# kellerberrin/KGL_Gene

Measured on AMD Instinct MI355X. Metric: variants·genomes/sec (allele-freq sweep), higher is better.
Workload: dtype u32

## Files before the change

### kgl_gene_amd/csrc/kgx_inbreed.hip

```cpp
#include <hip/hip_runtime.h>

#include <algorithm>
#include <cmath>
#include <cstdio>
#include <cstdlib>
#include <cstring>
#include <new>
#include <random>
#include <string>
#include <vector>

#include "kgx_kernels_inbreed.h"
#include "kgx_kernels_hall.h"
#include "kgx_kernels_loglik.h"
#include <hipcub/hipcub.hpp>
#include "kgx_internal.h"
#include "kgx_inbreed_plan.h"
#include "kgx_inbreed_buffers.h"

namespace kgx {
namespace {

int require_runtime(std::shared_ptr<Runtime>& rt) {
  rt = current_runtime();
  if (!rt) return fail(KGX_ENODEVICE, "kgx_init() has not succeeded: no gfx950 device bound (there is no CPU fallback)");
  return KGX_OK;
}

int sync_shards(const kgx_gt8* h) {
  for (const auto& sh : h->shards) {
    if (int rc = use_device(*sh.dev)) return rc;
    KGX_HIP(hipStreamSynchronize(sh.dev->stream));
  }
  return use_device(*h->shards[0].dev);
}

void destroy_shards(kgx_gt8* h) {
  for (auto& sh : h->shards)
    if ((sh.d_gt || sh.d_wide || sh.d_wide_of_row) && use_device(*sh.dev) == KGX_OK) {
      if (sh.d_gt) (void)hipFree(sh.d_gt);
      if (sh.d_wide) (void)hipFree(sh.d_wide);
      if (sh.d_wide_of_row) (void)hipFree(sh.d_wide_of_row);
      sh.d_gt = nullptr; sh.d_wide = nullptr; sh.d_wide_of_row = nullptr;
    }
  if (!h->shards.empty()) (void)use_device(*h->shards[0].dev);
}


static_assert(kAlgoSimple == KGX_ALGO_SIMPLE && kAlgoRitlandLocus == KGX_ALGO_RITLAND_LOCUS && kAlgoHallME == KGX_ALGO_HALL_ME &&
              kAlgoLoglikelihood == KGX_ALGO_LOGLIKELIHOOD, "the plan's algorithms are kgx.h's");

InbreedSwitches read_switches(int algorithm) {
  InbreedSwitches sw;
  sw.generic = env_int("KGX_K5_GENERIC", 0) != 0;
  sw.no_eval_lut = env_int("KGX_K5_NO_EVAL_LUT", 0) != 0;
  sw.no_table_sweep = env_int("KGX_K5_NO_TABLE_SWEEP", 0) != 0;
  sw.no_swar16 = env_int("KGX_K5_NO_SWAR16", 0) != 0;
  sw.eval_gpl = env_int("KGX_K5_EVAL_GPL", 8);
  if (sw.eval_gpl != 4 && sw.eval_gpl != 8) sw.eval_gpl = 8;
  sw.blocks_per_cu = env_int("KGX_K5_BLOCKS_PER_CU", 8);
  sw.eval_resident = env_int("KGX_K5_EVAL_RESIDENT", 2);
  sw.eval_rounds = env_int("KGX_K5_EVAL_ROUNDS", 8);
  sw.sequential_min = env_int("KGX_K5_SEQUENTIAL_MIN", 1 << 16);
  sw.always_guard = env_int("KGX_K5_ALWAYS_GUARD", 0) != 0;
  sw.xcds = static_cast<uint32_t>(std::max(1, env_int("KGX_K5_XCDS", 1)));
  sw.time_small_calls = env_int("KGX_TIME_SMALL_CALLS", 0) != 0;
  sw.keep_scratch_gb = env_int("KGX_KEEP_SCRATCH_GB", -1);
  sw.no_wave = env_int("KGX_K7_NO_WAVE", 0) != 0;
  sw.wave_loci = std::min(kGenomeWaveLoci, std::max(1, env_int("KGX_K7_WAVE_LOCI", 1024)));
  sw.wave_genomes = std::max(1, env_int("KGX_K7_WAVE_GENOMES", algorithm == KGX_ALGO_HALL_ME ? 1024 : 512));
  sw.search_brent = env_str("KGX_K7_SEARCH") == "brent";
  sw.hall_passes = env_int("KGX_K7_HALL_PASSES", 0) != 0;
  sw.golden = env_int("KGX_K7_GOLDEN", 0) != 0;
  sw.estimate_start = env_int("KGX_K7_ESTIMATE_START", 0);
  sw.ll_passes = env_int("KGX_K7_LL_PASSES", 0) != 0;
  sw.ll_het_terms = env_int("KGX_K7_LL_HET_TERMS", 0) != 0;
  sw.ll_dense_per_1024 = env_int("KGX_K7_LL_DENSE_PER_1024", 0);
  sw.class_sweeps = env_int("KGX_K7_CLASS_SWEEPS", 0) != 0;
  sw.class_bytes = env_int("KGX_K7_CLASS_BYTES", 0) != 0;
  sw.order_one_lane = env_int("KGX_K7_ORDER_ONE_LANE", 0) != 0;
  sw.no_pair = env_int("KGX_K7_NO_PAIR", 0) != 0;
  sw.no_compact = env_int("KGX_K7_NO_COMPACT", 0) != 0;
  sw.compact_min_genomes = env_int("KGX_K7_COMPACT_MIN_GENOMES", 2048);
  sw.compact_min_cells = env_int("KGX_K7_COMPACT_MIN_CELLS", 1 << 26);
  sw.trace = env_int("KGX_K7_TRACE", 0) != 0;
  return sw;
}

struct ClassHits {
  unsigned long long* words = nullptr;
  uint64_t word_blocks = 0;
  bool by_bits = false;
  HallClassRows class_rows{};
};

struct EvalTarget {
  const uint32_t* gt;
  uint64_t dwords_per_row, g0, n;
  const uint32_t* index;
  double* f;
};

struct InbreedCall;

struct ActiveSet {
  uint64_t n_act = 0, g0 = 0, dwords_per_row = 0;
  const uint32_t* gt = nullptr;
  const uint32_t* index = nullptr;
  BrentState* brent = nullptr;
  double* f = nullptr;
  uint32_t* d_global = nullptr;
  std::vector<uint32_t> global_of;
  std::vector<BrentState> host_states;
  bool may_compact_now = false;
  int compaction_level = 0;
  void compact(InbreedCall& c, unsigned int running, bool whatever_the_size);
};

struct InbreedCall {
  Device& dev;
  kgx_gt8_shard& sh;
  hipStream_t st;
  InbreedShape shape;
  InbreedSwitches sw;
  InbreedPlan plan;
  const uint32_t* locus_index;
  const double* minor_af;
  const double* start;
  kgx_locus_results* out;
  double* objective_out;
// ... 380 lines not shown
                             m.moments, block_bins, words_per_block, class_out, hits.word_blocks, static_cast<uint32_t>(block_base_of_class & 7u));
        });
      });
    } else {
      const dim3 sweep_grid(class_items[k] * hall_chunks);
      auto sweep = [&](auto gpl_c, auto emit_c) {
        hipLaunchKernelGGL((k_hall_sweep<decltype(gpl_c)::value, decltype(emit_c)::value>), sweep_grid, dim3(kBlock), 0, st, gt32, dwords_per_row, g0, n,
                           m.padded_of(k), m.items_of(k), h_counters + 4 * k, hall_chunks, code, m.moments, m.item_blocks_of(k), block_bins, words_per_block,
                           class_out);
      };
      if (plan.eval_gpl == 8) with_bool(emit, [&](auto emit_c) { sweep(std::integral_constant<int, 8>{}, emit_c); });
      else sweep(std::integral_constant<int, 4>{}, std::false_type{});
    }
    hipLaunchKernelGGL(k_hall_merge, dim3(hall_merge_blocks, 256), dim3(kBlock), 0, st, m.moments, item_base, n, m.bins, m.bin_used(), k + 1u);
    try_hip(hipGetLastError(), KGX_EHIP, "hall moments launch");
  }
  loglik_classes.n = emit ? hall_classes : 0u;
  loglik_classes.block_bins = block_bins;
  loglik_classes.plain_words = (by_bits && hall_mfma) ? 1u : 0u;
  loglik_classes.word_blocks = hits.word_blocks;
  loglik_classes.dense = sw.ll_dense_per_1024 > 0 ? sw.ll_dense_per_1024 / 1024.0 : kLoglikDense;
  try_hip(hipEventRecord(dev.moments_end, st), KGX_EHIP, "hipEventRecord");
  moments_timed = true;
  hipLaunchKernelGGL(k_hall_used_bins, dim3(1), dim3(kBlock), 0, st, m.bin_used(), m.used(), m.totals());
  try_hip(hipGetLastError(), KGX_EHIP, "hall bins launch");
  return rc == KGX_OK;
}

void InbreedCall::iterate_one_launch() {
  const uint64_t n = shape.n, n_sel = shape.n_sel;
  const bool hall = shape.algorithm == KGX_ALGO_HALL_ME;
  const bool per_wave = n_sel <= static_cast<uint64_t>(sw.wave_loci) && n >= static_cast<uint64_t>(sw.wave_genomes);
  const uint32_t wave_grid = static_cast<uint32_t>(per_wave ? (n + kBlock / kWave - 1) / (kBlock / kWave) : n);
  const double* estimate = hall ? b.d_sums : sw.estimate_start ? b.d_sums : nullptr;
  const int threads = per_wave ? kWave : kBlock;
  int cells = per_wave ? 8 : 2;
  while (cells < 32 && n_sel > static_cast<uint64_t>(threads) * cells) cells *= 2;
  with_int<1, 2>(hall ? 1 : 2, [&](auto mode_c) {
    auto launch = [&](auto cells_c, auto threads_c) {
      hipLaunchKernelGGL((k_inbreed_iterate_genome<decltype(mode_c)::value, decltype(cells_c)::value, decltype(threads_c)::value>), dim3(wave_grid), dim3(kBlock),
                         0, st, sh.d_gt, sh.pitch, shape.g0, n, d_index, n_sel, b.d_table, b.d_valid, shape.amax, shape.phased, b.d_counts, estimate, plan.search,
                         b.d_start, b.d_f, b.d_running);
    };
    if (per_wave) with_int<8, 16, 32>(cells, [&](auto cells_c) { launch(cells_c, std::integral_constant<int, kWave>{}); });
    else with_int<2, 4, 8, 16, 32>(cells, [&](auto cells_c) { launch(cells_c, std::integral_constant<int, kBlock>{}); });
  });
  wave_evaluations = !hall;
  dev.last_path = KGX_PATH_ONE_LAUNCH;
}

bool InbreedCall::hall_by_moments() {
  if (!(plan.hall_candidate && rc == KGX_OK && gather_moments(false))) return false;
  try_hip(hipEventRecord(dev.search_begin, st), KGX_EHIP, "hipEventRecord");
  hipLaunchKernelGGL(k_hall_iterate, dim3(static_cast<uint32_t>(shape.n)), dim3(kBlock), 0, st, m.bins, m.used(), m.totals(), b.d_counts, shape.n, b.d_start, b.d_f);
  try_hip(hipGetLastError(), KGX_EHIP, "hall iterate launch");
  try_hip(hipEventRecord(dev.search_end, st), KGX_EHIP, "hipEventRecord");
  search_timed = true;
  if (rc == KGX_OK) dev.last_path = KGX_PATH_HALL_MOMENTS;
  return rc == KGX_OK;
}

void InbreedCall::hall_by_passes() {
  const uint64_t n = shape.n, n_sel = shape.n_sel;
  if (rc == KGX_OK) dev.last_path = KGX_PATH_HALL_PASSES;
  const std::vector<double>& f0 = start_points;
  const unsigned long long walked =
      plan.eval_lut && n_sel ? (plan.eval_n_seg - 1) * plan.eval_per_seg + (n_sel - (plan.eval_n_seg - 1) * plan.eval_per_seg + 7) / 8 * 8 : 0ull;
  try_hip(hipMemcpyAsync(b.d_f, f0.data(), n * sizeof(double), hipMemcpyHostToDevice, st), KGX_EHIP, "H2D(f0)");
  try_hip(hipStreamSynchronize(st), KGX_EHIP, "sync");
  tabulate(1);
  std::vector<double> trace_prev, trace_prev2, trace_now;
  if (sw.trace) { trace_prev = f0; trace_prev2 = f0; trace_now.resize(n); }
  for (int it = 0; it < 50 && rc == KGX_OK; ++it) {
    estimator_pass(1, false);
    hipLaunchKernelGGL(k_reduce_parts, dim3(reduce_grid(n)), dim3(kBlock), 0, st, b.d_part, plan.pass_n_seg, n, nullptr, b.d_eval);
    hipLaunchKernelGGL(k_hall_update, dim3(lin_grid), dim3(kBlock), 0, st, b.d_eval, b.d_counts, n, walked, b.d_f);
    if (!sw.trace) continue;
    try_hip(hipMemcpyAsync(trace_now.data(), b.d_f, n * sizeof(double), hipMemcpyDeviceToHost, st), KGX_EHIP, "D2H(trace)");
    try_hip(hipStreamSynchronize(st), KGX_EHIP, "sync");
    uint64_t changed = 0, cycling = 0;
    double worst = 0.0;
    for (uint64_t g = 0; g < n; ++g) {
      if (trace_now[g] != trace_prev[g]) {
        ++changed;
        if (trace_now[g] == trace_prev2[g]) ++cycling;
        const double d = std::fabs(trace_now[g] - trace_prev[g]);
        worst = d > worst ? d : worst;
      }
    }
    std::fprintf(stderr, "[kgx] HallME step %d: %llu of %llu genomes moved (%llu back to the value before), largest move %.3e\n", it + 1,
                 (unsigned long long)changed, (unsigned long long)n, (unsigned long long)cycling, worst);
    trace_prev2 = trace_prev;
    trace_prev = trace_now;
  }
}

bool InbreedCall::loglik_by_moments(std::vector<uint32_t>& handed_over) {
  const uint64_t n = shape.n;
  const int objective_method = shape.objective_method;
  const bool loglik_moments = plan.loglik_candidate;
  if (objective_method == 1 && !loglik_moments)
    rc = fail(KGX_ESTATE, "kgx_inbreed_objective: this call would not run on the moments (selection size, amax, phase, memory or a switch)");
  if (!(loglik_moments && objective_method != 2 && rc == KGX_OK && gather_moments(true))) {
    if (objective_method == 1 && rc == KGX_OK)
      rc = fail(KGX_ESTATE, "kgx_inbreed_objective: a frequency without a bin, or no room for the hits' words: the passes would run");
    return false;
  }
  uint32_t* const h_totals = m.totals();
  uint32_t n_used = 0;
  try_hip(hipMemcpyAsync(&n_used, h_totals, sizeof(uint32_t), hipMemcpyDeviceToHost, st), KGX_EHIP, "D2H(used bins)");
  try_hip(hipStreamSynchronize(st), KGX_EHIP, "sync");
  unsigned long long* d_search_stats = sw.trace ? m.d_search_stats : nullptr;
  if (d_search_stats) try_hip(hipMemsetAsync(d_search_stats, 0, 8 * sizeof(unsigned long long), st), KGX_EHIP, "memset(search stats)");
  try_hip(hipEventRecord(dev.search_begin, st), KGX_EHIP, "hipEventRecord");
  hipLaunchKernelGGL(k_loglik_search, dim3(static_cast<uint32_t>(n)), dim3(kBlock), loglik_search_lds(n_used), st, m.bins, m.used(), h_totals, b.d_counts, b.d_sums,
                     m.d_smallest_het, n, plan.words_per_block, loglik_classes, b.d_start, objective_method == 1 ? 1 : 0, b.d_f, m.d_needs_passes, h_totals + 2,
                     b.d_running, d_search_stats);
  try_hip(hipGetLastError(), KGX_EHIP, "loglik search launch");
  try_hip(hipEventRecord(dev.search_end, st), KGX_EHIP, "hipEventRecord");
  search_timed = true;
  uint32_t handed = 0;
  unsigned int evaluations = 0;
  try_hip(hipMemcpyAsync(&handed, h_totals + 2, sizeof(uint32_t), hipMemcpyDeviceToHost, st), KGX_EHIP, "D2H(handed over)");
  try_hip(hipMemcpyAsync(&evaluations, b.d_running, sizeof(unsigned int), hipMemcpyDeviceToHost, st), KGX_EHIP, "D2H(evaluations)");
  try_hip(hipStreamSynchronize(st), KGX_EHIP, "sync");
  if (rc != KGX_OK) return false;
  if (d_search_stats) {
    unsigned long long stats[8] = {0};
    try_hip(hipMemcpy(stats, d_search_stats, sizeof(stats), hipMemcpyDeviceToHost), KGX_EHIP, "D2H(search stats)");
    std::fprintf(stderr, "kgx: Loglikelihood search over %llu genomes (%u bins used): %llu evaluations, %llu with cells in their band -- %llu served by kept cells, "
                         "%llu gathers kept, %llu gathers not kept, %llu dense walks; %llu cells listed, %llu blocks looked at\n",
                 (unsigned long long)n, n_used, stats[0], stats[1], stats[2], stats[3], stats[4], stats[5], stats[6], stats[7]);
  }
  dev.last_evaluations = static_cast<int>(evaluations);
  dev.last_path = KGX_PATH_LOGLIK_MOMENTS;
  if (handed) {
    std::vector<uint32_t> flags(n);
    try_hip(hipMemcpyAsync(flags.data(), m.d_needs_passes, n * sizeof(uint32_t), hipMemcpyDeviceToHost, st), KGX_EHIP, "D2H(needs passes)");
    try_hip(hipMemcpyAsync(b.d_keep, b.d_f, n * sizeof(double), hipMemcpyDeviceToDevice, st), KGX_EHIP, "copy(kept results)");
    try_hip(hipMemsetAsync(b.d_running, 0, sizeof(unsigned int), st), KGX_EHIP, "memset(running)");
    try_hip(hipStreamSynchronize(st), KGX_EHIP, "sync");
    for (uint64_t g = 0; g < n; ++g)
      if (flags[g]) {
        handed_over.push_back(static_cast<uint32_t>(g));
        if (sw.trace) std::fprintf(stderr, "kgx: Loglikelihood: genome %llu handed to the passes (reason %u)\n", (unsigned long long)(shape.g0 + g), flags[g]);
      }
    if (rc == KGX_OK) dev.last_path = KGX_PATH_LOGLIK_MOMENTS_AND_PASSES;
  }
  return true;
}

int InbreedCall::loglik_objective() {
  const uint64_t n = shape.n;
  if (shape.objective_method == 2 && rc == KGX_OK) {
    try_hip(hipMemcpyAsync(b.d_f, b.d_start, n * sizeof(double), hipMemcpyDeviceToDevice, st), KGX_EHIP, "copy(points)");
    tabulate(2);
    estimator_pass(2, false);
    hipLaunchKernelGGL(k_reduce_parts, dim3(reduce_grid(n)), dim3(kBlock), 0, st, b.d_part, plan.pass_n_seg, n, nullptr, b.d_eval);
    try_hip(hipGetLastError(), KGX_EHIP, "objective pass launch");
  }
  try_hip(hipMemcpyAsync(objective_out, shape.objective_method == 2 ? b.d_eval : b.d_f, n * sizeof(double), hipMemcpyDeviceToHost, st), KGX_EHIP, "D2H(objective)");
  try_hip(hipStreamSynchronize(st), KGX_EHIP, "sync");
  return rc;
}

void ActiveSet::compact(InbreedCall& c, unsigned int running, bool whatever_the_size) {
  Device& dev = c.dev;
  hipStream_t st = c.st;
  const uint64_t n_sel = c.shape.n_sel, planes = c.plan.planes;
  const uint64_t new_pitch = (static_cast<uint64_t>(running) + 127) / 128 * 128;
// ... 684 lines not shown
```

### kgl_gene_amd/csrc/kgx_inbreed_constants.h

```cpp
#ifndef KGX_INBREED_CONSTANTS_H
#define KGX_INBREED_CONSTANTS_H

#include <stdint.h>

#if defined(__HIPCC__)
#define KGX_HOST_DEVICE __host__ __device__
#else
#define KGX_HOST_DEVICE
#endif

namespace kgx {

constexpr int kWave = 64;
constexpr int kBlock = 256;

constexpr int kEvalBatch = 8;
constexpr uint64_t kRitlandSegment = 4088;

constexpr int kSearchBrent = 0, kSearchNelderMead = 1;
constexpr int kSearchNelderMeadPair = 2;

constexpr int kGenomeLoci = 8192;
constexpr int kGenomeWaveLoci = 2048;

constexpr int kHallMoments = 5;
constexpr int kHallKeyMantissa = 7;
constexpr int kHallMinExponent = -20;
constexpr uint32_t kHallBins = 1u + static_cast<uint32_t>(-kHallMinExponent) * (1u << kHallKeyMantissa) + 1u;
constexpr uint32_t kHallItemLoci = 2048;
struct HallRecord { uint32_t row; uint32_t bin; double delta; };
constexpr uint32_t kHallBlockLoci = 64;
constexpr uint64_t kBitsSpanGenomes = 2048;
constexpr uint64_t kBitsSpanBytes = kBitsSpanGenomes / 8;
KGX_HOST_DEVICE inline uint64_t hall_bit_row_bytes(uint64_t n_genomes) { return (n_genomes + kBitsSpanGenomes - 1) / kBitsSpanGenomes * kBitsSpanBytes; }

}

#endif
```

### kgl_gene_amd/csrc/kgx_inbreed_plan.h

```cpp
#ifndef KGX_INBREED_PLAN_H
#define KGX_INBREED_PLAN_H

#include <cassert>
#include <cstddef>
#include <stdint.h>

#include "kgx_inbreed_constants.h"

namespace kgx {

constexpr int kAlgoRitlandLocus = 0, kAlgoSimple = 1, kAlgoHallME = 2, kAlgoLoglikelihood = 3;

struct InbreedSwitches {
  bool generic = false;
  bool no_eval_lut = false;
  bool no_table_sweep = false;
  bool no_swar16 = false;
  int eval_gpl = 8;
  int blocks_per_cu = 8;
  int eval_resident = 2;
  int eval_rounds = 8;
  int sequential_min = 1 << 16;
  bool always_guard = false;
  uint32_t xcds = 1;
  bool time_small_calls = false;
  int keep_scratch_gb = -1;
  bool no_wave = false;
  int wave_loci = 1024;
  int wave_genomes = 1024;
  bool search_brent = false;
  bool hall_passes = false;
  bool golden = false;
  int estimate_start = 0;
  bool ll_passes = false;
  bool ll_het_terms = false;
  int ll_dense_per_1024 = 0;
  bool class_sweeps = false;
  bool class_bytes = false;
  bool order_one_lane = false;
  bool no_pair = false;
  bool no_compact = false;
  int compact_min_genomes = 2048;
  int compact_min_cells = 1 << 26;
  bool trace = false;
};

struct InbreedShape {
  uint64_t n = 0;
  uint64_t g0 = 0;
  uint64_t n_sel = 0;
  uint32_t amax = 1;
  int phased = 0;
  int algorithm = kAlgoSimple;
  int objective_method = 0;
  bool has_locus_index = false;
  int compute_units = 0;
};

struct InbreedPlan {
  bool ritland = false, table_sweep = false, swar16 = false, generic_sweep = false, eval_lut = false;
  int eval_gpl = 8;
  uint32_t gx = 0, gx16 = 0;
  uint64_t n_seg = 1, per_seg = 8, eval_n_seg = 1, eval_per_seg = 8, max_seg = 1, pass_n_seg = 1;
  bool sequential_defaults = false, wave_sized = false, table_passes = false;
  int search = kSearchNelderMead, pass_search = kSearchNelderMead;
  uint64_t planes = 1;
  bool hall_candidate = false, loglik_candidate = false;
  uint32_t hall_classes = 1;
  uint64_t hall_items = 0, hall_blocks = 0;
  uint64_t words_per_block = 0;
  bool hall_mfma = false, hall_bits_planned = false;
  bool hit_words_planned = false;
  uint64_t sel_pitch = 0, bit_row_bytes = 0;
  uint64_t moments_extra_bytes = 0;

  bool by_moments() const { return hall_candidate || loglik_candidate; }
  void take_the_passes() {
    hall_candidate = loglik_candidate = hall_mfma = hall_bits_planned = hit_words_planned = false;
    hall_items = hall_blocks = 0;
  }
};

inline InbreedPlan plan_inbreed(const InbreedShape& s, const InbreedSwitches& sw) {
  InbreedPlan p;
  const uint64_t n = s.n, g0 = s.g0, n_sel = s.n_sel;
  const uint32_t amax = s.amax;
  const uint64_t compute_units = static_cast<uint64_t>(s.compute_units);
  p.ritland = s.algorithm == kAlgoRitlandLocus;
  const bool no_tables = sw.generic || sw.no_eval_lut;
// ... 75 lines not shown
```

### kgl_gene_amd/csrc/kgx_kernels_hall.h

```cpp
#pragma once

#include <cstdint>

#include "kgx_kernels_inbreed.h"

namespace kgx {

constexpr uint32_t kHallNoKey = 0xFFFu;
constexpr int kHallBinsPerThread = (kHallBins + kBlock - 1) / kBlock;
static_assert(kHallBins < kHallNoKey, "12-bit sort keys");

struct HallItem { uint32_t begin, end, bin, pad; };
__host__ __device__ inline uint64_t hall_word_index(uint64_t block, uint64_t g, uint64_t lanes) {
  return ((block * 4 + ((g >> 1) & 3)) * lanes + (g >> 3)) * 2 + (g & 1);
}

__device__ __forceinline__ uint32_t hall_key(double y) {
  if (y == 0.0) return 0u;
  const uint64_t bits = static_cast<uint64_t>(__double_as_longlong(y));
  const int exponent = static_cast<int>((bits >> 52) & 0x7FFu) - 1023;
  if (!(y > 0.0) || exponent < kHallMinExponent || y > 1.0) return kHallNoKey;
  return 1u + static_cast<uint32_t>(exponent - kHallMinExponent) * (1u << kHallKeyMantissa) +
         static_cast<uint32_t>((bits >> (52 - kHallKeyMantissa)) & ((1u << kHallKeyMantissa) - 1u));
}
// ... 714 lines not shown
}

template <int BINS>
__device__ __forceinline__ double hall_iterate_genome(const double* __restrict__ bins, const uint32_t* __restrict__ used, uint32_t n_used,
                                                      uint64_t n_genomes, uint64_t g, double total, double F, double (&row_part)[2][16]) {
  double centre[BINS], m[BINS][kHallMoments];
#pragma unroll
  for (int i = 0; i < BINS; ++i) {
    const uint32_t at = threadIdx.x + static_cast<uint32_t>(i) * kBlock;
    centre[i] = 1.0;
#pragma unroll
    for (int j = 0; j < kHallMoments; ++j) m[i][j] = 0.0;
    if (at < n_used) {
      const uint32_t bin = used[at];
      centre[i] = hall_centre(bin);
#pragma unroll
      for (int j = 0; j < kHallMoments; ++j) m[i][j] = bins[(static_cast<uint64_t>(bin) * kHallMoments + j) * n_genomes + g];
    }
  }
  auto block_sum = [&](double v, int pass) {
    v = row_sum16(v);
    if ((threadIdx.x & 15) == 0) row_part[pass & 1][threadIdx.x >> 4] = v;
    __syncthreads();
    const double* p = row_part[pass & 1];
    double pair[8];
#pragma unroll
    for (int i = 0; i < 8; ++i) pair[i] = p[2 * i] + p[2 * i + 1];
    return ((pair[0] + pair[1]) + (pair[2] + pair[3])) + ((pair[4] + pair[5]) + (pair[6] + pair[7]));
  };
  for (int it = 0; it < 50; ++it) {
    const bool positive = F > 0.0;
    const double Fs = positive ? F : 1.0;
    const double u = 1.0 - Fs;
    double sum = 0.0;
#pragma unroll
    for (int i = 0; i < BINS; ++i) {
      const double q = 1.0 / __builtin_fma(u, centre[i], Fs);
      const double t = -u * q;
      double h = m[i][4];
      h = __builtin_fma(h, t, m[i][3]);
      h = __builtin_fma(h, t, m[i][2]);
      h = __builtin_fma(h, t, m[i][1]);
      h = __builtin_fma(h, t, m[i][0]);
      sum = __builtin_fma(q, h, sum);
    }
    const double S = block_sum(sum, it);
    F = positive ? (F * S) / total : 0.0 / total;
  }
  return F;
}

__global__ void __launch_bounds__(kBlock)
k_hall_iterate(const double* __restrict__ bins, const uint32_t* __restrict__ used, const uint32_t* __restrict__ n_used_ptr,
               const unsigned long long* __restrict__ counts, uint64_t n_genomes, const double* __restrict__ start, double* __restrict__ f_out) {
  __shared__ double row_part[2][16];
  const uint64_t g = blockIdx.x;
  if (g >= n_genomes) return;
  const uint32_t n_used = *n_used_ptr;
  const double total = static_cast<double>(counts[g * 6 + 4]);
  double F;
  if (n_used <= 4u * kBlock) F = hall_iterate_genome<4>(bins, used, n_used, n_genomes, g, total, start[g], row_part);
  else if (n_used <= 8u * kBlock) F = hall_iterate_genome<8>(bins, used, n_used, n_genomes, g, total, start[g], row_part);
  else F = hall_iterate_genome<kHallBinsPerThread>(bins, used, n_used, n_genomes, g, total, start[g], row_part);
  if (threadIdx.x == 0) f_out[g] = F;
}

}
```

### kgl_gene_amd/csrc/kgx_kernels_loglik.h

```cpp
#pragma once

#include <cstdint>

#include "kgx_kernels_hall.h"

namespace kgx {

constexpr int kLoglikTmaxLog2 = 4;
constexpr double kLoglikTmax = 1.0 / (1 << kLoglikTmaxLog2);
constexpr double kLoglikBand = 1.0 / (1.0 - (1.0 / 256.0) / kLoglikTmax);
constexpr double kLoglikReach = 0.5 * kLoglikBand * (1.0 + 1.0 / 64.0);
constexpr int kLoglikMaxClasses = 15;
constexpr uint32_t kLoglikListCells = 2560;
constexpr int kLoglikWordsPerThread = 4;
constexpr double kLoglikDense = 1.0 / 4.0;
constexpr double kLogSmallProb = -23.025850929940457;
constexpr int kLoglikBinValues = 6;

struct LoglikClass {
  const double* ys;
  const uint32_t* bin_block;
  const unsigned long long* words;
};
struct LoglikClasses { LoglikClass of[kLoglikMaxClasses]; uint32_t n; uint32_t block_bins; uint32_t plain_words; uint64_t word_blocks; double dense; };

inline size_t loglik_search_lds(uint32_t n_used) {
  return static_cast<size_t>(n_used) * (kLoglikBinValues * sizeof(double) + sizeof(uint32_t)) + 8;
}

__global__ void __launch_bounds__(kBlock)
k_loglik_search(const double* __restrict__ bins, const uint32_t* __restrict__ used, const uint32_t* __restrict__ n_used_ptr,
                const unsigned long long* __restrict__ counts, const double* __restrict__ sums,
                const unsigned long long* __restrict__ smallest_het, uint64_t n_genomes, uint64_t words_per_block, LoglikClasses classes,
                const double* __restrict__ start, int mode, double* __restrict__ f_out, uint32_t* __restrict__ needs_passes,
                uint32_t* __restrict__ handed_over, unsigned int* __restrict__ max_evaluations, unsigned long long* __restrict__ stats = nullptr) {
  extern __shared__ double bin_values[];
  __shared__ double row_part[2][3][16];
  __shared__ double cell_y[kLoglikListCells];
  __shared__ uint32_t wave_total[2][kBlock / kWave];
  const uint64_t g = blockIdx.x;
  if (g >= n_genomes) return;
  const uint32_t n_used = *n_used_ptr;
  uint32_t* const bin_keys = reinterpret_cast<uint32_t*>(bin_values + static_cast<size_t>(kLoglikBinValues) * n_used);
  for (uint32_t i = threadIdx.x; i < n_used; i += kBlock) {
    const uint32_t bin = used[i];
    const double* m = bins + static_cast<uint64_t>(bin) * kHallMoments * n_genomes + g;
    double v[kLoglikBinValues] = {m[0], 0.0, 0.0, 0.0, 0.0, 0.0};
    if (bin != 0u) {
      const double r = 1.0 / hall_centre(bin);
      v[1] = m[n_genomes]; v[2] = m[2 * n_genomes] * 0.5; v[3] = m[3 * n_genomes] * (1.0 / 3.0); v[4] = m[4 * n_genomes] * 0.25;
      v[5] = r * (v[1] - r * (v[2] - r * (v[3] - r * v[4])));
    }
#pragma unroll
    for (int j = 0; j < kLoglikBinValues; ++j) bin_values[static_cast<size_t>(j) * n_used + i] = v[j];
    bin_keys[i] = bin;
  }
  __syncthreads();
  const uint32_t wave = threadIdx.x / kWave, lane = threadIdx.x % kWave;
  const uint64_t lanes = words_per_block / 8;
  int pass = 0, scans = 0;
  auto block_sum3 = [&](double& a, double& b, double& c) {
    a = row_sum16(a);
    b = row_sum16(b);
    c = row_sum16(c);
    double (*slot)[16] = row_part[pass & 1];
    if ((threadIdx.x & 15) == 0) { slot[0][threadIdx.x >> 4] = a; slot[1][threadIdx.x >> 4] = b; slot[2][threadIdx.x >> 4] = c; }
    __syncthreads();
    double out[3];
#pragma unroll
    for (int which = 0; which < 3; ++which) {
      const double* p = slot[which];
      double pair[8];
#pragma unroll
      for (int i = 0; i < 8; ++i) pair[i] = p[2 * i] + p[2 * i + 1];
      out[which] = ((pair[0] + pair[1]) + (pair[2] + pair[3])) + ((pair[4] + pair[5]) + (pair[6] + pair[7]));
    }
    a = out[0]; b = out[1]; c = out[2];
    ++pass;
  };
  auto block_scan = [&](uint32_t mine, uint32_t& total) {
    uint32_t inclusive = mine;
#pragma unroll
    for (int off = 1; off < kWave; off <<= 1) {
      const uint32_t up = __shfl_up(inclusive, off);
      if (lane >= static_cast<uint32_t>(off)) inclusive += up;
    }
    uint32_t* totals = wave_total[scans & 1];
    if (lane == kWave - 1) totals[wave] = inclusive;
    __syncthreads();
    uint32_t before = 0;
    total = 0;
#pragma unroll
    for (uint32_t w = 0; w < kBlock / kWave; ++w) {
      if (w < wave) before += totals[w];
      total += totals[w];
    }
    ++scans;
    return before + inclusive - mine;
  };
  const unsigned long long sixth = counts[g * 6 + 5], total_cells = counts[g * 6 + 4];
  const double het_big = static_cast<double>(sixth >> 32);
  const double het_tiny = static_cast<double>(total_cells - (sixth & 0xFFFFFFFFull));
  const double het_cells = static_cast<double>(counts[g * 6 + 1] + counts[g * 6 + 3]) - het_tiny;
  const double het_term = sums[g * kParts0 + 4];
  const double w_smallest = __longlong_as_double(static_cast<long long>(*smallest_het));
  uint32_t hand_over = het_big != 0.0 ? 1u : 0u;

  auto band_of = [&](double F, uint32_t& key_lo, uint32_t& key_hi) {
    const double u = 1.0 - F;
    const double disc = sqrt(__builtin_fma(F, F, 4.0 * u * 1e-10));
    const double y_floor = u > 0.0 ? (F <= 0.0 ? (disc - F) / (2.0 * u) : 2e-10 / (F + disc)) : 1e-10;
    const double y_under = y_floor * (1.0 - 1e-9), y_over = y_floor * (1.0 + 1e-9);
    key_lo = y_under < 9.5367431640625e-07 ? 1u : hall_key(y_under);
    key_hi = y_over < 9.5367431640625e-07 ? 1u : hall_key(y_over) + 1u;
    const double edge = F < 0.0 ? -F / u * kLoglikBand : 0.0;
    if (edge >= 9.5367431640625e-07) {
      const uint32_t k_edge = hall_key(edge);
      const uint32_t from = hall_centre(k_edge) < edge ? k_edge + 1u : k_edge;
      key_hi = from > key_hi ? from : key_hi;
    }
  };
  uint32_t kept_lo = 0, kept_hi = 0, kept_n = 0;

  auto objective = [&](double F, double reach_lo, double reach_hi) -> double {
    const double u = 1.0 - F;
    uint32_t key_lo, key_hi, wide_lo, wide_hi, unused;
    band_of(F, key_lo, key_hi);
    band_of(reach_hi, wide_lo, unused);
    band_of(reach_lo, unused, wide_hi);
    wide_lo = wide_lo < key_lo ? wide_lo : key_lo;
    wide_hi = wide_hi > key_hi ? wide_hi : key_hi;
    double sum = 0.0, band_cells = 0.0, wide_cells = 0.0;
    for (uint32_t i = threadIdx.x; i < n_used; i += kBlock) {
      const uint32_t key = bin_keys[i];
      const double m0 = bin_values[i];
      if (key >= key_hi) {
        const double c = hall_centre(key);
        const double A = __builtin_fma(u, c, F), t = u / A;
        const double m1 = bin_values[n_used + i], m2 = bin_values[2 * n_used + i], m3 = bin_values[3 * n_used + i], m4 = bin_values[4 * n_used + i];
        sum += __builtin_fma(m0, log(c * A), bin_values[5 * n_used + i]) + t * (m1 - t * (m2 - t * (m3 - t * m4)));
      } else if (key < key_lo) {
        sum += m0 * kLogSmallProb;
      } else {
        band_cells += m0;
      }
      if (key >= wide_lo && key < wide_hi) wide_cells += m0;
    }
    block_sum3(sum, band_cells, wide_cells);
    double value = sum;
    if (stats && threadIdx.x == 0) { atomicAdd(stats + 0, 1ull); if (band_cells > 0.0) atomicAdd(stats + 1, 1ull); }
    if (band_cells > 0.0) {
      if (key_hi > classes.block_bins || wide_hi > classes.block_bins) hand_over = 2u;
      double prod = 1.0;
      int expo = 0;
      auto exact_cell = [&](double y) {
        const double yy = y * y, d = y - yy;
        const double p = __builtin_fmin(__builtin_fmax(__builtin_fma(F, d, yy), 0.0), 1.0);
        prod *= __builtin_fmax(p, 1e-10);
      };
      auto peel = [&]() {
        expo += __builtin_amdgcn_frexp_exp(prod);
        prod = __builtin_amdgcn_frexp_mant(prod);
      };
      const bool kept_covers = kept_hi != 0u && kept_lo <= key_lo && key_hi <= kept_hi;
      const bool keep = !kept_covers && wide_cells <= static_cast<double>(kLoglikListCells);
      const uint32_t from = keep ? wide_lo : key_lo, to = keep ? wide_hi : key_hi;
      uint32_t band_blocks = 0;
      if (!kept_covers)
        for (uint32_t k = 0; k < classes.n; ++k) band_blocks += classes.of[k].bin_block[to] - classes.of[k].bin_block[from];
      const bool dense = !kept_covers && !keep && band_cells >= classes.dense * static_cast<double>(band_blocks) * kHallBlockLoci;
      auto walk_listed = [&](uint32_t n_listed) {
        for (uint32_t i0 = 0; i0 < n_listed; i0 += 8 * kBlock) {
#pragma unroll
          for (int q = 0; q < 8; ++q) {
            const uint32_t i = i0 + static_cast<uint32_t>(q) * kBlock + threadIdx.x;
            if (i < n_listed) {
              const double y = cell_y[i];
              const uint32_t key = hall_key(y);
              if (key >= key_lo && key < key_hi) exact_cell(y);
            }
          }
          peel();
        }
      };
      if (stats && threadIdx.x == 0) {
        atomicAdd(stats + (kept_covers ? 2 : dense ? 5 : keep ? 3 : 4), 1ull);
        if (!kept_covers) atomicAdd(stats + 7, static_cast<unsigned long long>(band_blocks));
      }
      if (kept_covers) {
        walk_listed(kept_n);
      } else if (dense) {
        for (uint32_t k = 0; k < classes.n && !hand_over; ++k) {
          const LoglikClass& cl = classes.of[k];
          const uint32_t b0 = cl.bin_block[key_lo], b1 = cl.bin_block[key_hi];
          for (uint32_t b = b0 + 4u * wave; b < b1; b += 16u) {
            unsigned long long word[4];
            double y[4];
#pragma unroll
            for (int q = 0; q < 4; ++q) {
              const bool in = b + q < b1;
              word[q] = in ? cl.words[classes.plain_words ? g * classes.word_blocks + (b + q) : hall_word_index(b + q, g, lanes)] : 0ull;
              y[q] = cl.ys[static_cast<uint64_t>(in ? b + q : b0) * kHallBlockLoci + lane];
            }
#pragma unroll
            for (int q = 0; q < 4; ++q)
              if ((word[q] >> (63u - lane)) & 1ull) exact_cell(y[q]);
            peel();
          }
        }
      } else {
        uint32_t listed = 0;
        kept_hi = 0u;
        uint32_t* const cell_slot = reinterpret_cast<uint32_t*>(cell_y);
        for (uint32_t k = 0; k < classes.n && !hand_over; ++k) {
          const double* const class_ys = classes.of[k].ys;
          const unsigned long long* const class_words = classes.of[k].words;
          const uint32_t b0 = classes.of[k].bin_block[from], b1 = classes.of[k].bin_block[to];
          uint32_t converted = listed;
          auto fetch_frequencies = [&]() {
            for (uint32_t i = converted + threadIdx.x; i < listed; i += kBlock) cell_y[i] = class_ys[cell_slot[2u * i]];
            converted = listed;
          };
          auto load_words = [&](uint32_t base, unsigned long long (&word)[kLoglikWordsPerThread]) {
#pragma unroll
            for (int w = 0; w < kLoglikWordsPerThread; ++w) {
              const uint32_t b = base + static_cast<uint32_t>(w) * kBlock + threadIdx.x;
              word[w] = b < b1 ? class_words[classes.plain_words ? g * classes.word_blocks + b : hall_word_index(b, g, lanes)] : 0ull;
            }
          };
          unsigned long long next_word[kLoglikWordsPerThread];
          if (b0 < b1) load_words(b0, next_word);
          for (uint32_t base = b0; base < b1; base += kBlock * kLoglikWordsPerThread) {
            unsigned long long word[kLoglikWordsPerThread];
            uint32_t mine = 0;
#pragma unroll
            for (int w = 0; w < kLoglikWordsPerThread; ++w) word[w] = next_word[w];
            if (base + kBlock * kLoglikWordsPerThread < b1) load_words(base + kBlock * kLoglikWordsPerThread, next_word);
#pragma unroll
            for (int w = 0; w < kLoglikWordsPerThread; ++w) mine += static_cast<uint32_t>(__popcll(word[w]));
            uint32_t round_total = 0;
            uint32_t at = listed + block_scan(mine, round_total);
            bool to_list = true;
            if (listed + round_total > kLoglikListCells) {
              if (keep) { hand_over = 4u; break; }
              __syncthreads();
              fetch_frequencies();
              __syncthreads();
              walk_listed(listed);
              __syncthreads();
              at -= listed;
              listed = 0;
              converted = 0;
              to_list = round_total <= kLoglikListCells;
            }
#pragma unroll
            for (int w = 0; w < kLoglikWordsPerThread; ++w) {
              const uint32_t first = (base + static_cast<uint32_t>(w) * kBlock + threadIdx.x) * kHallBlockLoci;
              unsigned long long bits = word[w];
              int walked = 0;
              while (bits != 0ull) {
                const int p = __clzll(static_cast<long long>(bits));
                bits &= ~(0x8000000000000000ull >> p);
                if (to_list) cell_slot[2u * at++] = first + static_cast<uint32_t>(p);
                else { exact_cell(class_ys[first + static_cast<uint32_t>(p)]); if ((++walked & 7) == 0) peel(); }
              }
              if (!to_list) peel();
            }
            if (to_list) listed += round_total;
          }
          __syncthreads();
          fetch_frequencies();
        }
        __syncthreads();
        if (stats && threadIdx.x == 0) atomicAdd(stats + 6, static_cast<unsigned long long>(listed));
        if (keep && !hand_over) {
          if (static_cast<double>(listed) != wide_cells) hand_over = 4u;
          kept_lo = from; kept_hi = to; kept_n = listed;
        }
        walk_listed(listed);
        if (!keep) __syncthreads();
      }
      double exact = log(prod) + static_cast<double>(expo) * 0.6931471805599453, nothing = 0.0, none = 0.0;
      block_sum3(exact, nothing, none);
      value += exact;
    }
    value += het_tiny * kLogSmallProb;
    if (het_cells > 0.0) {
      if (u * w_smallest >= 1.0000001e-10) value += het_term + het_cells * log(u);
      else if (u <= 2e-10) value += het_cells * kLogSmallProb;
      else hand_over = 3u;
    }
    return value;
  };

  if (mode == 1) {
    const double v = objective(start[g], start[g], start[g]);
    if (threadIdx.x == 0) {
      f_out[g] = hand_over ? __builtin_nan("") : v;
      needs_passes[g] = hand_over;
      if (hand_over) atomicAdd(handed_over, 1u);
    }
    return;
  }
  BrentState s = nm_start(start[g]);
  unsigned int evaluations = 0;
  for (int it = 0; it < 500 && !hand_over; ++it) {
    const double F = it == 0 ? s.x : s.u;
    const double lo = s.a < s.b ? s.a : s.b, hi = s.a < s.b ? s.b : s.a;
    const double value = objective(F, lo < F ? lo : F, hi > F ? hi : F);
    ++evaluations;
    if (hand_over) break;
    nm_advance(s, value);
    if (s.done) break;
  }
  if (threadIdx.x == 0) {
    f_out[g] = hand_over ? __builtin_nan("") : s.x;
    needs_passes[g] = hand_over;
    if (hand_over) atomicAdd(handed_over, 1u);
    atomicMax(max_evaluations, evaluations);
  }
}

__global__ void __launch_bounds__(kBlock)
k_loglik_keep(const uint32_t* __restrict__ needs_passes, const double* __restrict__ kept, uint64_t n, int planes, BrentState* __restrict__ st,
              double* __restrict__ f_next) {
  for (uint64_t g = static_cast<uint64_t>(blockIdx.x) * blockDim.x + threadIdx.x; g < n; g += static_cast<uint64_t>(gridDim.x) * blockDim.x) {
    if (needs_passes[g]) continue;
    BrentState s = st[g];
    s.done = 1;
    s.x = kept[g];
    st[g] = s;
    for (int k = 0; k < planes; ++k) f_next[k * n + g] = kept[g];
  }
}

}
```

Measured before the change: 25320 billion.

## Remap workgroups across XCDs, defer wide-band sum, and force wave-uniform values in loglik search

Adds an XCD-aware mapping from workgroup to genome in the Hall and loglik search kernels, so neighbouring genomes share a chiplet and its cache. The loglik search now computes the wide-band cell count only when a band is occupied and the kept list does not already cover it, which removes one reduction from every evaluation. Class descriptors are staged in LDS, word indexing is precomputed, and readfirstlane and asm barriers pin scalar and vector placement to cut register pressure and redundant loads. A tunable list-cell cap is also added. These changes add complexity and could alter floating-point ordering or uniformity assumptions.

```diff
diff --git a/kgl_gene_amd/csrc/kgx_inbreed.hip b/kgl_gene_amd/csrc/kgx_inbreed.hip
--- a/kgl_gene_amd/csrc/kgx_inbreed.hip
+++ b/kgl_gene_amd/csrc/kgx_inbreed.hip
@@ -76,6 +76,7 @@
   sw.ll_passes = env_int("KGX_K7_LL_PASSES", 0) != 0;
   sw.ll_het_terms = env_int("KGX_K7_LL_HET_TERMS", 0) != 0;
   sw.ll_dense_per_1024 = env_int("KGX_K7_LL_DENSE_PER_1024", 0);
+  sw.ll_list_cells = env_int("KGX_K7_LL_LIST_CELLS", 0);
   sw.class_sweeps = env_int("KGX_K7_CLASS_SWEEPS", 0) != 0;
   sw.class_bytes = env_int("KGX_K7_CLASS_BYTES", 0) != 0;
   sw.order_one_lane = env_int("KGX_K7_ORDER_ONE_LANE", 0) != 0;
@@ -562,7 +563,8 @@
 bool InbreedCall::hall_by_moments() {
   if (!(plan.hall_candidate && rc == KGX_OK && gather_moments(false))) return false;
   try_hip(hipEventRecord(dev.search_begin, st), KGX_EHIP, "hipEventRecord");
-  hipLaunchKernelGGL(k_hall_iterate, dim3(static_cast<uint32_t>(shape.n)), dim3(kBlock), 0, st, m.bins, m.used(), m.totals(), b.d_counts, shape.n, b.d_start, b.d_f);
+  hipLaunchKernelGGL(k_hall_iterate, dim3(static_cast<uint32_t>(shape.n)), dim3(kBlock), 0, st, m.bins, m.used(), m.totals(), b.d_counts, shape.n, b.d_start, b.d_f,
+                     sw.xcds);
   try_hip(hipGetLastError(), KGX_EHIP, "hall iterate launch");
   try_hip(hipEventRecord(dev.search_end, st), KGX_EHIP, "hipEventRecord");
   search_timed = true;
@@ -621,11 +623,12 @@
   try_hip(hipMemcpyAsync(&n_used, h_totals, sizeof(uint32_t), hipMemcpyDeviceToHost, st), KGX_EHIP, "D2H(used bins)");
   try_hip(hipStreamSynchronize(st), KGX_EHIP, "sync");
   unsigned long long* d_search_stats = sw.trace ? m.d_search_stats : nullptr;
+  const uint32_t list_cells = sw.ll_list_cells > 0 && sw.ll_list_cells < static_cast<int>(kLoglikListCells) ? static_cast<uint32_t>(sw.ll_list_cells) : kLoglikListCells;
   if (d_search_stats) try_hip(hipMemsetAsync(d_search_stats, 0, 8 * sizeof(unsigned long long), st), KGX_EHIP, "memset(search stats)");
   try_hip(hipEventRecord(dev.search_begin, st), KGX_EHIP, "hipEventRecord");
   hipLaunchKernelGGL(k_loglik_search, dim3(static_cast<uint32_t>(n)), dim3(kBlock), loglik_search_lds(n_used), st, m.bins, m.used(), h_totals, b.d_counts, b.d_sums,
                      m.d_smallest_het, n, plan.words_per_block, loglik_classes, b.d_start, objective_method == 1 ? 1 : 0, b.d_f, m.d_needs_passes, h_totals + 2,
-                     b.d_running, d_search_stats);
+                     b.d_running, sw.xcds, list_cells, d_search_stats);
   try_hip(hipGetLastError(), KGX_EHIP, "loglik search launch");
   try_hip(hipEventRecord(dev.search_end, st), KGX_EHIP, "hipEventRecord");
   search_timed = true;
diff --git a/kgl_gene_amd/csrc/kgx_inbreed_constants.h b/kgl_gene_amd/csrc/kgx_inbreed_constants.h
--- a/kgl_gene_amd/csrc/kgx_inbreed_constants.h
+++ b/kgl_gene_amd/csrc/kgx_inbreed_constants.h
@@ -34,6 +34,14 @@
 constexpr uint64_t kBitsSpanBytes = kBitsSpanGenomes / 8;
 KGX_HOST_DEVICE inline uint64_t hall_bit_row_bytes(uint64_t n_genomes) { return (n_genomes + kBitsSpanGenomes - 1) / kBitsSpanGenomes * kBitsSpanBytes; }
 
+constexpr uint32_t kLineGenomes = 8;
+KGX_HOST_DEVICE inline uint64_t genome_of_workgroup(uint64_t block, uint64_t n_genomes, uint32_t xcds) {
+  const uint64_t round = static_cast<uint64_t>(kLineGenomes) * xcds;
+  if (xcds <= 1u || block >= n_genomes / round * round) return block;
+  const uint64_t w = block % round;
+  return (block / round * xcds + w % xcds) * kLineGenomes + w / xcds;
+}
+
 }
 
 #endif
diff --git a/kgl_gene_amd/csrc/kgx_inbreed_plan.h b/kgl_gene_amd/csrc/kgx_inbreed_plan.h
--- a/kgl_gene_amd/csrc/kgx_inbreed_plan.h
+++ b/kgl_gene_amd/csrc/kgx_inbreed_plan.h
@@ -35,6 +35,7 @@
   bool ll_passes = false;
   bool ll_het_terms = false;
   int ll_dense_per_1024 = 0;
+  int ll_list_cells = 0;
   bool class_sweeps = false;
   bool class_bytes = false;
   bool order_one_lane = false;
diff --git a/kgl_gene_amd/csrc/kgx_kernels_hall.h b/kgl_gene_amd/csrc/kgx_kernels_hall.h
--- a/kgl_gene_amd/csrc/kgx_kernels_hall.h
+++ b/kgl_gene_amd/csrc/kgx_kernels_hall.h
@@ -790,10 +790,10 @@
 
 __global__ void __launch_bounds__(kBlock)
 k_hall_iterate(const double* __restrict__ bins, const uint32_t* __restrict__ used, const uint32_t* __restrict__ n_used_ptr,
-               const unsigned long long* __restrict__ counts, uint64_t n_genomes, const double* __restrict__ start, double* __restrict__ f_out) {
+               const unsigned long long* __restrict__ counts, uint64_t n_genomes, const double* __restrict__ start, double* __restrict__ f_out, uint32_t xcds) {
   __shared__ double row_part[2][16];
-  const uint64_t g = blockIdx.x;
-  if (g >= n_genomes) return;
+  if (blockIdx.x >= n_genomes) return;
+  const uint64_t g = genome_of_workgroup(blockIdx.x, n_genomes, xcds);
   const uint32_t n_used = *n_used_ptr;
   const double total = static_cast<double>(counts[g * 6 + 4]);
   double F;
diff --git a/kgl_gene_amd/csrc/kgx_kernels_loglik.h b/kgl_gene_amd/csrc/kgx_kernels_loglik.h
--- a/kgl_gene_amd/csrc/kgx_kernels_loglik.h
+++ b/kgl_gene_amd/csrc/kgx_kernels_loglik.h
@@ -28,18 +28,31 @@
   return static_cast<size_t>(n_used) * (kLoglikBinValues * sizeof(double) + sizeof(uint32_t)) + 8;
 }
 
+__device__ inline uint32_t wave_uniform(uint32_t v) { return static_cast<uint32_t>(__builtin_amdgcn_readfirstlane(static_cast<int>(v))); }
+__device__ inline unsigned long long wave_uniform(unsigned long long v) {
+  return (static_cast<unsigned long long>(wave_uniform(static_cast<uint32_t>(v >> 32))) << 32) | wave_uniform(static_cast<uint32_t>(v));
+}
+__device__ inline double wave_uniform(double v) { return __longlong_as_double(static_cast<long long>(wave_uniform(static_cast<unsigned long long>(__double_as_longlong(v))))); }
+template <typename T>
+__device__ inline const T* wave_uniform(const T* p) { return reinterpret_cast<const T*>(wave_uniform(static_cast<unsigned long long>(reinterpret_cast<uintptr_t>(p)))); }
+template <typename T>
+__device__ inline T in_lanes(T v) { asm volatile("" : "+v"(v)); return v; }
+
 __global__ void __launch_bounds__(kBlock)
 k_loglik_search(const double* __restrict__ bins, const uint32_t* __restrict__ used, const uint32_t* __restrict__ n_used_ptr,
                 const unsigned long long* __restrict__ counts, const double* __restrict__ sums,
                 const unsigned long long* __restrict__ smallest_het, uint64_t n_genomes, uint64_t words_per_block, LoglikClasses classes,
                 const double* __restrict__ start, int mode, double* __restrict__ f_out, uint32_t* __restrict__ needs_passes,
-                uint32_t* __restrict__ handed_over, unsigned int* __restrict__ max_evaluations, unsigned long long* __restrict__ stats = nullptr) {
+                uint32_t* __restrict__ handed_over, unsigned int* __restrict__ max_evaluations, uint32_t xcds, uint32_t list_cells_arg,
+                unsigned long long* __restrict__ stats = nullptr) {
   extern __shared__ double bin_values[];
-  __shared__ double row_part[2][3][16];
+  __shared__ double row_part[2][2][16];
   __shared__ double cell_y[kLoglikListCells];
   __shared__ uint32_t wave_total[2][kBlock / kWave];
-  const uint64_t g = blockIdx.x;
-  if (g >= n_genomes) return;
+  __shared__ LoglikClass class_of[kLoglikMaxClasses];
+  if (blockIdx.x >= n_genomes) return;
+  const uint64_t g = genome_of_workgroup(blockIdx.x, n_genomes, xcds);
+  if (threadIdx.x < classes.n) class_of[threadIdx.x] = classes.of[threadIdx.x];
   const uint32_t n_used = *n_used_ptr;
   uint32_t* const bin_keys = reinterpret_cast<uint32_t*>(bin_values + static_cast<size_t>(kLoglikBinValues) * n_used);
   for (uint32_t i = threadIdx.x; i < n_used; i += kBlock) {
@@ -57,25 +70,35 @@
   }
   __syncthreads();
   const uint32_t wave = threadIdx.x / kWave, lane = threadIdx.x % kWave;
-  const uint64_t lanes = words_per_block / 8;
+  const uint64_t word_step = in_lanes(classes.plain_words ? uint64_t{1} : hall_word_index(1, 0, words_per_block / 8));
+  const uint64_t word_first = in_lanes(classes.plain_words ? g * classes.word_blocks : hall_word_index(0, g, words_per_block / 8));
+  const uint32_t block_bins = in_lanes(classes.block_bins), list_size = in_lanes(list_cells_arg);
+  const double dense_from = in_lanes(classes.dense);
   int pass = 0, scans = 0;
-  auto block_sum3 = [&](double& a, double& b, double& c) {
+  auto block_sum1 = [&](double a, double (&slot)[16]) {
     a = row_sum16(a);
-    b = row_sum16(b);
-    c = row_sum16(c);
+    if ((threadIdx.x & 15) == 0) slot[threadIdx.x >> 4] = a;
+  };
+  auto block_sum_out = [&](const double (&slot)[16]) {
+    double pair[8];
+#pragma unroll
+    for (int i = 0; i < 8; ++i) pair[i] = slot[2 * i] + slot[2 * i + 1];
+    return wave_uniform(((pair[0] + pair[1]) + (pair[2] + pair[3])) + ((pair[4] + pair[5]) + (pair[6] + pair[7])));
+  };
+  auto block_sum = [&](double& a) {
     double (*slot)[16] = row_part[pass & 1];
-    if ((threadIdx.x & 15) == 0) { slot[0][threadIdx.x >> 4] = a; slot[1][threadIdx.x >> 4] = b; slot[2][threadIdx.x >> 4] = c; }
+    block_sum1(a, slot[0]);
     __syncthreads();
-    double out[3];
-#pragma unroll
-    for (int which = 0; which < 3; ++which) {
-      const double* p = slot[which];
-      double pair[8];
-#pragma unroll
-      for (int i = 0; i < 8; ++i) pair[i] = p[2 * i] + p[2 * i + 1];
-      out[which] = ((pair[0] + pair[1]) + (pair[2] + pair[3])) + ((pair[4] + pair[5]) + (pair[6] + pair[7]));
-    }
-    a = out[0]; b = out[1]; c = out[2];
+    a = block_sum_out(slot[0]);
+    ++pass;
+  };
+  auto block_sum2 = [&](double& a, double& b) {
+    double (*slot)[16] = row_part[pass & 1];
+    block_sum1(a, slot[0]);
+    block_sum1(b, slot[1]);
+    __syncthreads();
+    a = block_sum_out(slot[0]);
+    b = block_sum_out(slot[1]);
     ++pass;
   };
   auto block_scan = [&](uint32_t mine, uint32_t& total) {
@@ -96,14 +119,17 @@
       total += totals[w];
     }
     ++scans;
+    total = wave_uniform(total);
     return before + inclusive - mine;
   };
   const unsigned long long sixth = counts[g * 6 + 5], total_cells = counts[g * 6 + 4];
   const double het_big = static_cast<double>(sixth >> 32);
-  const double het_tiny = static_cast<double>(total_cells - (sixth & 0xFFFFFFFFull));
-  const double het_cells = static_cast<double>(counts[g * 6 + 1] + counts[g * 6 + 3]) - het_tiny;
-  const double het_term = sums[g * kParts0 + 4];
-  const double w_smallest = __longlong_as_double(static_cast<long long>(*smallest_het));
+  const double het_tiny = in_lanes(static_cast<double>(total_cells - (sixth & 0xFFFFFFFFull)));
+  const double het_cells = in_lanes(static_cast<double>(counts[g * 6 + 1] + counts[g * 6 + 3]) - het_tiny);
+  const double het_term = in_lanes(sums[g * kParts0 + 4]);
+  const double w_smallest = in_lanes(__longlong_as_double(static_cast<long long>(*smallest_het)));
+  f_out = in_lanes(f_out); needs_passes = in_lanes(needs_passes); handed_over = in_lanes(handed_over); max_evaluations = in_lanes(max_evaluations);
+  stats = in_lanes(stats);
   uint32_t hand_over = het_big != 0.0 ? 1u : 0u;
 
   auto band_of = [&](double F, uint32_t& key_lo, uint32_t& key_hi) {
@@ -124,13 +150,9 @@
 
   auto objective = [&](double F, double reach_lo, double reach_hi) -> double {
     const double u = 1.0 - F;
-    uint32_t key_lo, key_hi, wide_lo, wide_hi, unused;
+    uint32_t key_lo, key_hi;
     band_of(F, key_lo, key_hi);
-    band_of(reach_hi, wide_lo, unused);
-    band_of(reach_lo, unused, wide_hi);
-    wide_lo = wide_lo < key_lo ? wide_lo : key_lo;
-    wide_hi = wide_hi > key_hi ? wide_hi : key_hi;
-    double sum = 0.0, band_cells = 0.0, wide_cells = 0.0;
+    double sum = 0.0, band_cells = 0.0;
     for (uint32_t i = threadIdx.x; i < n_used; i += kBlock) {
       const uint32_t key = bin_keys[i];
       const double m0 = bin_values[i];
@@ -144,13 +166,27 @@
       } else {
         band_cells += m0;
       }
-      if (key >= wide_lo && key < wide_hi) wide_cells += m0;
-    }
-    block_sum3(sum, band_cells, wide_cells);
+    }
+    block_sum2(sum, band_cells);
     double value = sum;
     if (stats && threadIdx.x == 0) { atomicAdd(stats + 0, 1ull); if (band_cells > 0.0) atomicAdd(stats + 1, 1ull); }
     if (band_cells > 0.0) {
-      if (key_hi > classes.block_bins || wide_hi > classes.block_bins) hand_over = 2u;
+      const bool kept_covers = kept_hi != 0u && kept_lo <= key_lo && key_hi <= kept_hi;
+      uint32_t wide_lo = key_lo, wide_hi = key_hi;
+      double wide_cells = 0.0;
+      if (!kept_covers) {
+        uint32_t reach_key_lo, reach_key_hi, unused;
+        band_of(reach_hi, reach_key_lo, unused);
+        band_of(reach_lo, unused, reach_key_hi);
+        wide_lo = reach_key_lo < key_lo ? reach_key_lo : key_lo;
+        wide_hi = reach_key_hi > key_hi ? reach_key_hi : key_hi;
+        for (uint32_t i = threadIdx.x; i < n_used; i += kBlock) {
+          const uint32_t key = bin_keys[i];
+          if (key >= wide_lo && key < wide_hi) wide_cells += bin_values[i];
+        }
+        block_sum(wide_cells);
+      }
+      if (const uint32_t kept_bins = wave_uniform(block_bins); key_hi > kept_bins || wide_hi > kept_bins) hand_over = 2u;
       double prod = 1.0;
       int expo = 0;
       auto exact_cell = [&](double y) {
@@ -162,13 +198,16 @@
         expo += __builtin_amdgcn_frexp_exp(prod);
         prod = __builtin_amdgcn_frexp_mant(prod);
       };
-      const bool kept_covers = kept_hi != 0u && kept_lo <= key_lo && key_hi <= kept_hi;
-      const bool keep = !kept_covers && wide_cells <= static_cast<double>(kLoglikListCells);
+      const uint32_t list_cells = wave_uniform(list_size);
+      const bool keep = !kept_covers && wide_cells <= static_cast<double>(list_cells);
       const uint32_t from = keep ? wide_lo : key_lo, to = keep ? wide_hi : key_hi;
       uint32_t band_blocks = 0;
       if (!kept_covers)
-        for (uint32_t k = 0; k < classes.n; ++k) band_blocks += classes.of[k].bin_block[to] - classes.of[k].bin_block[from];
-      const bool dense = !kept_covers && !keep && band_cells >= classes.dense * static_cast<double>(band_blocks) * kHallBlockLoci;
+        for (uint32_t k = 0; k < classes.n; ++k) {
+          const uint32_t* const bin_block = wave_uniform(class_of[k].bin_block);
+          band_blocks += bin_block[to] - bin_block[from];
+        }
+      const bool dense = !kept_covers && !keep && band_cells >= wave_uniform(dense_from) * static_cast<double>(band_blocks) * kHallBlockLoci;
       auto walk_listed = [&](uint32_t n_listed) {
         for (uint32_t i0 = 0; i0 < n_listed; i0 += 8 * kBlock) {
 #pragma unroll
@@ -191,7 +230,7 @@
         walk_listed(kept_n);
       } else if (dense) {
         for (uint32_t k = 0; k < classes.n && !hand_over; ++k) {
-          const LoglikClass& cl = classes.of[k];
+          const LoglikClass cl{wave_uniform(class_of[k].ys), wave_uniform(class_of[k].bin_block), wave_uniform(class_of[k].words)};
           const uint32_t b0 = cl.bin_block[key_lo], b1 = cl.bin_block[key_hi];
           for (uint32_t b = b0 + 4u * wave; b < b1; b += 16u) {
             unsigned long long word[4];
@@ -199,7 +238,7 @@
 #pragma unroll
             for (int q = 0; q < 4; ++q) {
               const bool in = b + q < b1;
-              word[q] = in ? cl.words[classes.plain_words ? g * classes.word_blocks + (b + q) : hall_word_index(b + q, g, lanes)] : 0ull;
+              word[q] = in ? cl.words[(b + q) * word_step + word_first] : 0ull;
               y[q] = cl.ys[static_cast<uint64_t>(in ? b + q : b0) * kHallBlockLoci + lane];
             }
 #pragma unroll
@@ -213,9 +252,10 @@
         kept_hi = 0u;
         uint32_t* const cell_slot = reinterpret_cast<uint32_t*>(cell_y);
         for (uint32_t k = 0; k < classes.n && !hand_over; ++k) {
-          const double* const class_ys = classes.of[k].ys;
-          const unsigned long long* const class_words = classes.of[k].words;
-          const uint32_t b0 = classes.of[k].bin_block[from], b1 = classes.of[k].bin_block[to];
+          const double* const class_ys = wave_uniform(class_of[k].ys);
+          const unsigned long long* const class_words = wave_uniform(class_of[k].words);
+          const uint32_t* const bin_block = wave_uniform(class_of[k].bin_block);
+          const uint32_t b0 = bin_block[from], b1 = bin_block[to];
           uint32_t converted = listed;
           auto fetch_frequencies = [&]() {
             for (uint32_t i = converted + threadIdx.x; i < listed; i += kBlock) cell_y[i] = class_ys[cell_slot[2u * i]];
@@ -225,7 +265,7 @@
 #pragma unroll
             for (int w = 0; w < kLoglikWordsPerThread; ++w) {
               const uint32_t b = base + static_cast<uint32_t>(w) * kBlock + threadIdx.x;
-              word[w] = b < b1 ? class_words[classes.plain_words ? g * classes.word_blocks + b : hall_word_index(b, g, lanes)] : 0ull;
+              word[w] = b < b1 ? class_words[b * word_step + word_first] : 0ull;
             }
           };
           unsigned long long next_word[kLoglikWordsPerThread];
@@ -241,7 +281,7 @@
             uint32_t round_total = 0;
             uint32_t at = listed + block_scan(mine, round_total);
             bool to_list = true;
-            if (listed + round_total > kLoglikListCells) {
+            if (listed + round_total > list_cells) {
               if (keep) { hand_over = 4u; break; }
               __syncthreads();
               fetch_frequencies();
@@ -251,7 +291,7 @@
               at -= listed;
               listed = 0;
               converted = 0;
-              to_list = round_total <= kLoglikListCells;
+              to_list = round_total <= list_cells;
             }
 #pragma unroll
             for (int w = 0; w < kLoglikWordsPerThread; ++w) {
@@ -280,8 +320,8 @@
         walk_listed(listed);
         if (!keep) __syncthreads();
       }
-      double exact = log(prod) + static_cast<double>(expo) * 0.6931471805599453, nothing = 0.0, none = 0.0;
-      block_sum3(exact, nothing, none);
+      double exact = log(prod) + static_cast<double>(expo) * 0.6931471805599453;
+      block_sum(exact);
       value += exact;
     }
     value += het_tiny * kLogSmallProb;
@@ -290,7 +330,7 @@
       else if (u <= 2e-10) value += het_cells * kLogSmallProb;
       else hand_over = 3u;
     }
-    return value;
+    return wave_uniform(value);
   };
 
   if (mode == 1) {
@@ -302,16 +342,16 @@
     }
     return;
   }
-  BrentState s = nm_start(start[g]);
+  BrentState s = nm_start(in_lanes(start[g]));
   unsigned int evaluations = 0;
   for (int it = 0; it < 500 && !hand_over; ++it) {
-    const double F = it == 0 ? s.x : s.u;
-    const double lo = s.a < s.b ? s.a : s.b, hi = s.a < s.b ? s.b : s.a;
+    const double F = wave_uniform(it == 0 ? s.x : s.u);
+    const double sa = wave_uniform(s.a), sb = wave_uniform(s.b), lo = sa < sb ? sa : sb, hi = sa < sb ? sb : sa;
     const double value = objective(F, lo < F ? lo : F, hi > F ? hi : F);
     ++evaluations;
     if (hand_over) break;
-    nm_advance(s, value);
-    if (s.done) break;
+    nm_advance(s, in_lanes(value));
+    if (wave_uniform(static_cast<uint32_t>(s.done))) break;
   }
   if (threadIdx.x == 0) {
     f_out[g] = hand_over ? __builtin_nan("") : s.x;
```

New measurement: 25240 billion. No clear change (-0.3%).
